# sin0235/FaceRecognition

Hardware: AMD Instinct MI355X
Metric: aligned faces/sec (embed+match) ArcFace@112 bs=256, 1/2/4/8 MI355X (higher is better)
Workload: dtype bf16; 1 GPU; iresnet100 bf16 embed bs=256/GPU + top-5 match vs 10000x512 f32 gallery (row-sharded over 1 GPU(s)); batch_per_gpu=256, global_batch=256, gallery_rows=10000, k=5, parallelism=dp1

## Files before the change

### facerecognition_amd/csrc/engine.cpp

```cpp
#include <algorithm>
#include <cmath>
#include <cstdio>
#include <cstdlib>
#include <cstring>
#include <memory>
#include <mutex>
#include <string>
#include <unordered_map>
#include <vector>

#include "engine_internal.h"

namespace fr {
static thread_local std::string g_err;
void set_error(const std::string& m) { g_err = m; }

static const std::vector<std::pair<std::string, std::string>>& ab_table() {
    static const std::vector<std::pair<std::string, std::string>> t = [] {
        std::vector<std::pair<std::string, std::string>> r;
        const char* e = getenv("FR_AB");
        const std::string v = e ? e : "";
        size_t p = 0;
        while (p < v.size()) {
            size_t q = v.find(',', p);
// ... 427 lines not shown
        h->stages.push_back(r);
    }
};

std::string L(int l, int i) { return "layer" + std::to_string(l) + "." + std::to_string(i); }

void build_iresnet100(Builder& b) {
    fr_handle* h = b.h;
    h->in_size = 112;
    const int in = b.tensor(112, 112, 8);
    h->ops.push_back(Op{OP_PRE, -1, 0, 0, in});
    int x = b.tensor(112, 112, 64, "prelu");
    b.stem = true;
    b.conv({"conv1"}, in, 0, 8, x, 0, 3, 3, 1, 1, 1, 1, 2);
    h->ops[h->ops.size() - 2].fuse_stem = true;
    const int planes[4] = {64, 128, 256, 512}, nblk[4] = {3, 13, 30, 3};
    int H = 112, C = 64;
    StageRec tail_rec;
    int tail_st_op = -1;
    for (int l = 0; l < 4; ++l) {
        const int P = planes[l], Ho = H / 2;
        int st_op = -1;
        StageRec rec;
        auto close_stage = [&](bool layer_end) {
            if (st_op >= 0 && !b.rc && layer_end && !rec.fp8 &&
                ((l == 2 && rec.parts == 1 && rec.C == 256) || (l == 1 && rec.parts == 2 && rec.C == 128 && rec.H == 28))) {
                rec.out = x;
                rec.nblk = (int)rec.t_tensors.size();
                tail_rec = rec;
                tail_st_op = st_op;
            } else if (st_op >= 0) {
                rec.out = x;
                rec.nblk = (int)rec.t_tensors.size();
                b.close_stage(st_op, rec);
            }
            st_op = -1;
        };
        for (int i = 0; i < nblk[l]; ++i) {
            const bool s14 = stage_supported(1, Ho, Ho, P);
            const int parts = split_stage_parts(Ho, Ho, P);
            const std::string pre = L(l + 1, i);
            const bool f8 = b.is_fp8(pre + ".conv1") && b.is_fp8(pre + ".conv2");
            const bool mixed = b.is_fp8(pre + ".conv1") != b.is_fp8(pre + ".conv2");
            const bool can = i >= 1 && P == C && !mixed && (f8 ? s14 : (s14 || parts > 0));
            if (st_op >= 0 && (!can || f8 != rec.fp8)) close_stage(false);
            if (can && st_op < 0) {
                st_op = b.open_stage();
                rec = StageRec{};
                rec.kind = STAGE_LDS;
                rec.in = x;
                rec.parts = s14 ? 1 : parts;
                rec.H = Ho;
                rec.C = P;
                rec.fp8 = f8;
            }
            const int Hin = i == 0 ? H : Ho, st = i == 0 ? 2 : 1;
            const bool fuse = i == 0 && b.fuse_ds(P, C, pre);
            const bool tr = i == 0 && fuse && !b.is_fp8(pre + ".conv1") && !b.is_fp8(pre + ".conv2") &&
                            trans_supported(1, H, H, C, P, P, 9 * C, 9 * P + C);
            const int tr_op = tr ? b.open_stage() : -1;
            const int hmid = b.tensor(Hin, Hin, P, pre + ".prelu");
            b.conv({pre + ".conv1"}, x, 0, C, hmid, 0, 3, 3, 1, 1, 1, 1, 2);
            if (tail_st_op >= 0 && !b.rc) {
                const int oi = (int)h->ops.size() - 1;
                const Op& op = h->ops[oi];
                const DevConvW& cw = h->convw[op.wi];
                static const bool no_tail = ab_int("no_stage_tail", 0) != 0;
                const int TC = tail_rec.C;
                if (!no_tail && h->dtype != FR_DTYPE_FP8 && !cw.w8 && op.act == 2 && cw.slope && cw.Cout == 2 * TC &&
                    cw.Npad >= 2 * TC && cw.Cin == TC && cw.Kh == 3 && cw.Kw == 3 && op.sh == 1 && op.sw == 1 && op.ph == 1 &&
                    op.pw == 1 && op.in == tail_rec.out && op.in_off == 0 && op.out_off == 0 && op.res < 0 && op.x2 < 0 &&
                    op.out2 < 0 && h->tensors[hmid].C == 2 * TC && !h->tensors[hmid].f16)
                    tail_rec.tail_op = oi;
                if (tail_rec.tail_op >= 0) tail_rec.conv_ops.push_back(oi);
                b.close_stage(tail_st_op, tail_rec);
                tail_st_op = -1;
            }
// ... 2 lines not shown
                res = b.tensor(Ho, Ho, P, pre + ".downsample");
                b.conv({pre + ".downsample"}, x, 0, C, res, 0, 1, 1, 2, 2, 0, 0, 0);
            }
            const int y = b.tensor(Ho, Ho, P, pre);
            if (fuse)
                b.conv_ds({pre + ".conv2"}, hmid, 0, P, y, 0, 3, 3, st, st, 1, 1, 0, -1, 0, -1, "", pre + ".downsample",
                          x, C, 2);
            else
                b.conv({pre + ".conv2"}, hmid, 0, P, y, 0, 3, 3, st, st, 1, 1, 0, res, 0);
            if (tr && !b.rc) {
                StageRec t;
                t.kind = STAGE_TRANS;
                t.in = x; t.out = y; t.nblk = 1; t.H = H; t.C = P;
                t.conv_ops = {(int)h->ops.size() - 2, (int)h->ops.size() - 1};
                t.t_tensors = {hmid};
                t.x_tensors = {y};
                b.close_stage(tr_op, t);
            }
            if (st_op >= 0 && !b.rc) {
                rec.conv_ops.push_back((int)h->ops.size() - 2);
                rec.conv_ops.push_back((int)h->ops.size() - 1);
                rec.t_tensors.push_back(hmid);
                rec.x_tensors.push_back(y);
            }
            x = y;
            C = P;
        }
        close_stage(true);
        H = Ho;
    }
    b.head(x);
}

int build_img_weights(fr_handle* h) {
    for (const auto& op : h->ops) {
        if (op.kind != OP_CONV || op.wi < 0) continue;
        DevConvW& cw = h->convw[op.wi];
        if ((cw.wimg || cw.wrows) && cw.wring) continue;
        ConvArgs a{};
        a.B = 1; a.Cin = op.cin; a.Kh = op.kh; a.Kw = op.kw; a.sh = op.sh; a.sw = op.sw; a.ph = op.ph; a.pw = op.pw;
        a.H = h->tensors[op.in].H; a.W = h->tensors[op.in].W; a.Cx = h->tensors[op.in].C; a.x_off = op.in_off;
        a.Ho = h->tensors[op.out].H; a.Wo = h->tensors[op.out].W; a.Cy = h->tensors[op.out].C; a.y_off = op.out_off;
        a.Cout = cw.Cout; a.Npad = cw.Npad; a.Kpad = cw.Kpad; a.bias9 = cw.bias9;
        a.y2 = op.out2 >= 0 ? (bf16_t*)1 : nullptr;
        if (op.res >= 0) { a.res = (const bf16_t*)1; a.Cres = h->tensors[op.res].C; a.res_off = op.res_off; }
        a.f16 = h->dtype == FR_DTYPE_F16;
// ... 334 lines not shown
        if ((rc = dev_alloc(&q, FR_SPLITK_TILES * sizeof(int)))) { free_acts(h); return rc; }
        h->act_allocs.push_back(q);
        FR_HIP_CHECK(hipMemset(q, 0, FR_SPLITK_TILES * sizeof(int)));
        h->splitk_cnt = (int*)q;
    }
    h->max_batch = maxB;
    if (std::any_of(h->need_amax.begin(), h->need_amax.end(), [](char c) { return c != 0; })) {
        void* q = nullptr;
        rc = dev_alloc(&q, h->tensors.size() * FR_AMAX_SLOTS * sizeof(float));
        if (rc) { free_acts(h); return rc; }
        h->act_allocs.push_back(q);
        h->amax = (float*)q;
    }
    if (h->proj_d) {
        void* q = nullptr;
        rc = dev_alloc(&q, (size_t)maxB * h->embed_dim * sizeof(float));
        if (rc) { free_acts(h); return rc; }
        h->act_allocs.push_back(q);
        h->emb_pre = (float*)q;
    }
    if (std::any_of(h->stages.begin(), h->stages.end(), [](const StageRec& r) { return r.parts > 1; })) {
        if (h->stages.size() > FR_MAX_SPLIT_STAGES) { set_error("reserve: too many stage ops"); return FR_ERR_ARG; }
        void* q = nullptr;
        rc = dev_alloc(&q, split_stage_xchg_elems(maxB) * sizeof(bf16_t));
        if (rc) { free_acts(h); return rc; }
        h->act_allocs.push_back(q);
        h->stage_xchg = (bf16_t*)q;
        rc = dev_alloc(&q, (size_t)maxB * 4 * FR_MAX_SPLIT_STAGES * sizeof(int));
        if (rc) { free_acts(h); return rc; }
        h->act_allocs.push_back(q);
        FR_HIP_CHECK(hipMemset(q, 0, (size_t)maxB * 4 * FR_MAX_SPLIT_STAGES * sizeof(int)));
        h->stage_flags = (int*)q;
    }
    return fill_stage_dbg(h);
}

bool img28_enabled() {
    static const bool on = [] { return !ab_int("no_img28", 0); }();
    return on;
}

bool rows_enabled() {
    static const bool on = [] { return !ab_int("no_rows", 0); }();
    return on;
}

bool img56_enabled() {
// ... 1172 lines not shown
        case FR_OPT_X3_MIN_ROWS:
            if (value < 1) { set_error("fr_set_option: FR_OPT_X3_MIN_ROWS must be >= 1"); return FR_ERR_ARG; }
            h->x3_min_rows = value;
            break;
        case FR_OPT_STAGE_SPIN_LIMIT: h->spin_limit = value; break;
        case FR_OPT_STAGE_VARIANT:
            if (value < 0 || value > 3) { set_error("fr_set_option: FR_OPT_STAGE_VARIANT is 0 .. 3"); return FR_ERR_ARG; }
            h->stage_variant = value;
            break;
        case FR_OPT_SPLITK_INLAUNCH: h->splitk_inlaunch = value != 0; break;
        case FR_OPT_BATCH_INVARIANT:
            if (value != 0 && h->dtype == FR_DTYPE_FP8) {
                set_error("fr_set_option: FR_OPT_BATCH_INVARIANT is not available on FR_DTYPE_FP8 handles (their e4m3 "
                          "convs scale activations by a per-batch amax)");
                return FR_ERR_ARG;
            }
            if ((value != 0) != h->invariant) {
                h->invariant = value != 0;
                h->tuned.clear();
                h->tuned_batches.clear();
            }
            break;
        case FR_OPT_FUSED_MASK:
            if (value < 0 || value > 127) { set_error("fr_set_option: FR_OPT_FUSED_MASK is 0 .. 127"); return FR_ERR_ARG; }
            h->fused_mask = value;
            break;
        default: set_error("fr_set_option: unknown option " + std::to_string(option)); return FR_ERR_ARG;
    }
    drop_graphs(h);
    return FR_OK;
}

int fr_get_option(const fr_handle* h, int option) {
    if (!h) return FR_ERR_ARG;
    switch (option) {
        case FR_OPT_STAGE: return h->stages.empty() ? 0 : h->stage_mode;
        case FR_OPT_STAGE_MIN_FILL: return h->stage_min_fill;
        case FR_OPT_KEEP_INTERMEDIATES: return h->keep_inter ? 1 : 0;
        case FR_OPT_MATCH_EXACT: return h->match_exact ? 1 : 0;
        case FR_OPT_X3_MIN_ROWS: return (int)h->x3_min_rows;
        case FR_OPT_STAGE_SPIN_LIMIT: return h->spin_limit;
        case FR_OPT_STAGE_VARIANT: return h->stage_variant;
        case FR_OPT_SPLITK_INLAUNCH: return h->splitk_inlaunch ? 1 : 0;
        case FR_OPT_BATCH_INVARIANT: return h->invariant ? 1 : 0;
        case FR_OPT_FUSED_MASK: return h->fused_mask;
        default: return FR_ERR_ARG;
    }
// ... 574 lines not shown
```

### facerecognition_amd/csrc/engine_internal.h

```cpp
#pragma once
#include <mutex>
#include <string>
#include <vector>

#include "../../include/frhip.h"
#include "kernels.h"

#pragma GCC visibility push(hidden)

namespace fr {

struct DevConvW {
    bf16_t* w = nullptr;
    float* bias = nullptr;
    float* slope = nullptr;
    float* aff_s = nullptr;
    float* aff_b = nullptr;
    float* bias9 = nullptr;
    bf16_t* wimg = nullptr;
    float* negf = nullptr;
    bf16_t* wrows = nullptr;
    float* ep = nullptr;
    bf16_t* wring = nullptr;
    uint8_t* w8 = nullptr;
// ... 16 lines not shown
    int in = -1, in_off = 0, cin = 0;
    int out = -1, out_off = 0;
    int res = -1, res_off = 0;
    int out2 = -1;
    int kh = 1, kw = 1, sh = 1, sw = 1, ph = 0, pw = 0;
    int act = 0;
    int wi = -1;
    int pk = 0, ps = 0, pp = 0;
    int stage = -1;
    int x2 = -1, x2_off = 0, st2 = 1;
    bool fuse_stem = false;
    int grp = -1;
};

enum StageKind {
    STAGE_LDS,
    STAGE_TRANS,
    STAGE_STEM160,
    STAGE_CHAIN35,
    STAGE_CHAIN17,
    STAGE_CHAIN_R50,
    STAGE_BNECK28,
    STAGE_STEM_R50,
    STAGE_NKINDS
};

struct StageRec {
    StageKind kind = STAGE_LDS;
    int in = -1, out = -1, nblk = 0;
    int parts = 1, H = 14, C = 256;
    std::vector<int> conv_ops;
    std::vector<int> t_tensors, x_tensors;
    bf16_t* w = nullptr;
    StageConv* table = nullptr;
    float* ep = nullptr;
    float* slope = nullptr;
    bf16_t** dbg = nullptr;
    bool fp8 = false;
    uint8_t* w8 = nullptr;
    float* wscale = nullptr;
    int tail_op = -1;
    bf16_t* tw1 = nullptr;
    bf16_t* tw2 = nullptr;
    float* tep1 = nullptr;
    float* tsl1 = nullptr;
    float* tb2 = nullptr;
// ... 68 lines not shown
    float* proj_b = nullptr;
    int proj_d = 0;
    float* emb_pre = nullptr;
    float* amax = nullptr;
    std::vector<char> need_amax;
    bf16_t* stage_xchg = nullptr;
    int* stage_flags = nullptr;
    int* stage_spin = nullptr;
    int* fail_host = nullptr;
    int* fail_dev = nullptr;
    int spin_limit = 0;
    int stage_variant = 0;
    bool no_split = false;
    int64_t stage_reruns = 0;
    hipEvent_t chk_ev = nullptr;
    hipEvent_t async_ev = nullptr;
    bool async_pending = false;
    bool split_registered = false;
    int stage_mode = 1;
    int stage_min_fill = 80;
    int n_cu = 256;
    bool keep_inter = false;
    bool invariant = false;
    int fused_mask = 127;
    const uint8_t* fwd_u8 = nullptr;
};

#pragma GCC visibility push(hidden)

namespace fr {

int dev_alloc(void** p, size_t bytes);

template <class T>
int upload(fr_handle* h, T** dst, const std::vector<T>& src) {
    void* p = nullptr;
    int rc = dev_alloc(&p, src.size() * sizeof(T));
    if (rc) return rc;
    h->weight_allocs.push_back(p);
    FR_HIP_CHECK(hipMemcpy(p, src.data(), src.size() * sizeof(T), hipMemcpyHostToDevice));
    *dst = (T*)p;
    return FR_OK;
}

int run_conv_op(fr_handle* h, const Op& op, int B, int f16, hipStream_t s);
int run_maxpool_op(fr_handle* h, const Op& op, int B, int f16, hipStream_t s);

// ... 62 lines not shown
```

### facerecognition_amd/csrc/kernels.h

```cpp
#pragma once
#include "common.h"

namespace fr {

enum { TILE_128x128 = 0, TILE_256x64 = 1, TILE_128x64 = 2, TILE_64x128 = 3,
       TILE_128x128_S3 = 4, TILE_256x128 = 5, TILE_128x256 = 6,
       TILE_128x64_S3 = 8, TILE_64x128_S3 = 9, NUM_TILE_IDS = 10,
       TILE_WRING = 13,
       TILE_DIRECT = 14,
       TILE_64x64_S3 = 17, TILE_64x64 = 18, TILE_32x64_S3 = 19 };

struct ConvArgs {
    const bf16_t* x; int B, H, W, Cx, x_off, Cin;
    const bf16_t* w; int Kh, Kw, sh, sw, ph, pw, K, Kpad;
    int Ho, Wo, M, Cout, Npad;
    const float* bias; const float* slope; int act;
    const float* bias9;
    const bf16_t* res; int Cres, res_off;
    bf16_t* y; int Cy, y_off;
    bf16_t* y2; int Cy2, y2_off; const float* aff_s; const float* aff_b;
    float* partial; int split_k;
    int f16;
    int tile;
    void* ev0;
// ... 69 lines not shown
    int* flags;
    int* spin_timeouts;
    int* fail_host;
    int spin_limit;
    int variant;
    int ntail;
    bf16_t* y2;
    int B, nblk, f16;
    void* ev0;
    void* ev1;
};
bool stage_supported(int B, int H, int W, int C);
size_t stage_weight_bytes(int nconv);
void stage_pack_weights(const bf16_t* rows, int Kpad, int C, bf16_t* out);
hipError_t launch_stage(const StageArgs& a, hipStream_t s);
size_t stage8_weight_bytes(int nconv);
void stage8_pack_weights(const uint8_t* rows, int Kpad8, uint8_t* out);
hipError_t launch_stage8(const StageArgs& a, hipStream_t s);
int split_stage_parts(int H, int W, int C);
size_t split_stage_weight_bytes(int C, int nconv);
void split_stage_pack_weights(const bf16_t* rows, int Kpad, int C, bf16_t* out);
size_t split_stage_xchg_elems(int B);
hipError_t launch_split_stage(const StageArgs& a, int H, int C, hipStream_t s);
struct TransArgs {
    const bf16_t* x;
    bf16_t* y;
    const bf16_t* w1;
    const bf16_t* w2;
    const float* ep1;
    const float* slope1;
    const float* b2;
    int B, f16;
    void* ev0;
    void* ev1;
};
bool trans_supported(int B, int H, int W, int Cin, int Cmid, int Cout, int K1, int K2);
size_t trans_packed_elems(int K);
hipError_t trans_pack_weights(const bf16_t* w, int Kpad, int K, bf16_t* out, hipStream_t s);
hipError_t launch_trans(const TransArgs& a, hipStream_t s);
struct Chain17Args {
    const bf16_t* x;
    bf16_t* y;
    const bf16_t* w;
    const float* bias;
    int B, nblk, f16;
    void* ev0;
// ... 130 lines not shown
```

### facerecognition_amd/csrc/stages.cpp

```cpp
#include <algorithm>
#include <cstdio>

#include "engine_internal.h"

namespace fr {

struct StageKindDesc {
    const char* name;
    int mask_bit;
    const char* ab_off[2];
    const char* ab_off_split;
    bool keeps_inter;
    bool no_amax;
    bool takes_u8;
    bool per_block;
    const char* cls;
    const char* label;
    const char* ksize;
    int pix, N, K;
    int K_ds;
};

static const StageKindDesc kinds[STAGE_NKINDS] = {
     {"stage", 1, {nullptr, nullptr}, "no_split_stage", true, false, false, false, nullptr, "stage", "3x3", 0, 0, 0, 0},
     {"transition", 1, {"no_trans", nullptr}, nullptr, false, true, false, false, "trans layer1.0", "trans", "3x3", 3136, 64, 2944, 0},
     {"stem160", 2, {"no_stem160", nullptr}, nullptr, false, false, true, false, "stem160", "stem160", "3x3", 1, 1, 185697536, 0},
     {"chain35", 4, {"no_chain", "no_chain35"}, nullptr, false, false, false, false, "chain block35", "chain", "3x3", 289, 256, 300, 0},
     {"chain", 8, {"no_chain", "no_chain17"}, nullptr, false, false, false, false, "chain block17", "chain", "1x1", 64, 896, 768, 0},
     {"chain_r50", 16, {"no_chain", "no_chain50"}, nullptr, false, false, false, false, "chain r50 layer3", "chain", "3x3", 49, 1024, 1088, 0},
     {"bneck28", 32, {"no_chain", "no_bneck28"}, nullptr, false, false, false, true, nullptr, "chain", "3x3", 784, 256, 272, 288},
     {"stem_r50", 64, {"no_chain", "no_stem_r50"}, nullptr, false, false, true, false, "stem r50", "chain", "7x7", 3136, 64, 392, 0},
};

struct StageWork {
    int pix, N, K, units;
};

static StageWork stage_work(const StageRec& r, int i) {
    const StageKindDesc& d = kinds[r.kind];
    StageWork w = {d.pix, d.N, d.K, r.nblk};
    if (!d.pix) w = {r.H * r.H, r.C, 9 * r.C, 2 * r.nblk};
    if (d.per_block && i >= 0) {
        w.units = 1;
        if (r.bn_ds && i == 0) w.K = d.K_ds;
    }
    return w;
}

static double stage_bytes(const fr_handle* h, const StageRec& r, const StageWork& w, int B, int i) {
    const double in_px = h->fwd_u8 ? 3.0 : 16.0;
    switch (r.kind) {
        case STAGE_TRANS: return 2.0 * B * (12544.0 + 3136.0) * 64 + 2.0 * 64 * (576 + 640);
        case STAGE_STEM160: return (double)B * (in_px * 160 * 160 + 2.0 * 38 * 38 * 80);
        case STAGE_STEM_R50: return (double)B * (112.0 * 112 * in_px + 28.0 * 28 * 64 * 2);
        case STAGE_BNECK28: return 2.0 * B * w.pix * ((r.bn_ds && i == 0 ? 64.0 : 256.0) + w.N) + 2.0 * w.N * w.K;
        default: return 2.0 * 2.0 * B * w.pix * w.N + (r.fp8 ? 1.0 : 2.0) * w.N * w.K * w.units;
    }
}

static const char* stage_class(const StageRec& r, int i) {
    switch (r.kind) {
        case STAGE_LDS: return r.fp8 ? "stage8 layer3" : r.H == 14 ? "stage layer3" : r.H == 28 ? "stage layer2" : "stage layer1";
        case STAGE_BNECK28: return r.bn_ds && i == 0 ? "bneck28 layer1.0" : "bneck28 layer1";
        default: return kinds[r.kind].cls;
// ... 83 lines not shown
        FR_HIP_CHECK(hipMemcpy(slope.data(), cw.slope, cw.Cout * sizeof(float), hipMemcpyDeviceToHost));
        for (int hf = 0; hf < 2; ++hf) {
            const int c = nconv + hf;
            if (r.parts > 1) split_stage_pack_weights(rows.data() + (size_t)hf * C * cw.Kpad, cw.Kpad, C, packed.data() + c * per);
            else stage_pack_weights(rows.data() + (size_t)hf * C * cw.Kpad, cw.Kpad, C, packed.data() + c * per);
            for (int k = 0; k < 9; ++k)
                std::copy(b9.begin() + (size_t)k * cw.Npad + hf * C, b9.begin() + (size_t)k * cw.Npad + hf * C + C,
                          ep.begin() + ((size_t)c * 9 + k) * C);
            std::copy(slope.begin() + hf * C, slope.begin() + hf * C + C, sl.begin() + (size_t)c * C);
        }
    }
    int rc = r.fp8 ? upload(h, &r.w8, packed8) : upload(h, &r.w, packed);
    if (rc) return rc;
    if (r.fp8 && (rc = upload(h, &r.wscale, wsc))) return rc;
    rc = upload(h, &r.table, tab);
    if (rc) return rc;
    if ((rc = upload(h, &r.ep, ep))) return rc;
    if ((rc = upload(h, &r.slope, sl))) return rc;
    void* d = nullptr;
    if ((rc = dev_alloc(&d, (size_t)nconv * sizeof(bf16_t*)))) return rc;
    h->weight_allocs.push_back(d);
    r.dbg = (bf16_t**)d;
    if (r.parts > 1 && !h->stage_spin) {
        if ((rc = dev_alloc(&d, sizeof(int)))) return rc;
        h->weight_allocs.push_back(d);
        h->stage_spin = (int*)d;
        FR_HIP_CHECK(hipMemset(h->stage_spin, 0, sizeof(int)));
    }
    return FR_OK;
}

int fill_stage_dbg(fr_handle* h) {
    for (auto& r : h->stages) {
        if (!kinds[r.kind].keeps_inter) continue;
        std::vector<bf16_t*> p(2 * r.nblk);
        for (int i = 0; i < r.nblk; ++i) {
            p[i] = h->tensors[r.x_tensors[i]].dev;
            p[r.nblk + i] = h->tensors[r.t_tensors[i]].dev;
        }
        FR_HIP_CHECK(hipMemcpy(r.dbg, p.data(), p.size() * sizeof(bf16_t*), hipMemcpyHostToDevice));
    }
    return FR_OK;
}

static int build_trans(fr_handle* h, StageRec& r) {
    const DevConvW& c1 = h->convw[h->ops[r.conv_ops[0]].wi];
// ... 176 lines not shown
        }
        bool shapes = cw[0]->Cout == 96 && cw[0]->K == 256 && cw[0]->Kh == 1 && cw[4]->Cout == 256 && cw[4]->K == 96 &&
                      cw[4]->Kh == 1 && op[4]->res >= 0 && op[4]->res_off == 0;
        for (int k = 1; k <= 3; ++k)
            shapes = shapes && cw[k]->Cout == 32 && cw[k]->K == 288 && cw[k]->Kh == 3 && cw[k]->Kw == 3 && op[k]->ph == 1 &&
                     op[k]->pw == 1 && op[k]->sh == 1 && op[k]->res < 0;
        if (!shapes) return bad_shapes("chain35 member convs do not have Block35's shapes");
        chain35_pack_block(m[0].rows.data(), cw[0]->Kpad, m[1].rows.data(), cw[1]->Kpad, m[2].rows.data(), cw[2]->Kpad,
                           m[3].rows.data(), cw[3]->Kpad, m[4].rows.data(), cw[4]->Kpad, blk, packed.data());
        chain35_pack_bias(m[0].bias.data(), m[1].bias.data(), m[2].bias.data(), m[3].bias.data(), m[4].bias.data(), blk,
                          bias.data());
    }
    return chain_upload(h, r, packed, bias);
}

int pack_stage(fr_handle* h, StageRec& r) {
    switch (r.kind) {
        case STAGE_LDS: return build_stage(h, r);
        case STAGE_TRANS: return build_trans(h, r);
        case STAGE_CHAIN35: return build_chain35(h, r);
        case STAGE_CHAIN17: return build_chain17(h, r);
        case STAGE_CHAIN_R50: return build_chain_r50(h, r);
        case STAGE_BNECK28: return build_bneck28(h, r);
        default: return FR_OK;
    }
}

int stage_choice(const fr_handle* h, int st, int B) {
    for (const auto& m : h->stage_meas)
        if (m.stage == st && m.B == B) return m.run;
    return -1;
}

static bool stage_runs(const fr_handle* h, int B, const StageRec& r, int st) {
    const StageKindDesc& d = kinds[r.kind];
    if (h->stage_mode == 0 || h->invariant) return false;
    if (!(h->fused_mask & d.mask_bit)) return false;
    if (h->keep_inter && !d.keeps_inter) return false;
    if (d.no_amax && h->amax && h->need_amax[r.out]) return false;
    if (!kind_enabled(r) || (r.parts > 1 && h->no_split)) return false;
    if (h->stage_mode == 1) {
        const int c = stage_choice(h, st, B);
        if (c >= 0) return c == 1;
    }
    const int cap = std::max(1, h->n_cu / r.parts);
    if (h->stage_mode == 2 || B <= cap) return true;
    const int64_t rounds = (B + cap - 1) / cap;
    return (int64_t)B * 100 >= (int64_t)h->stage_min_fill * rounds * cap;
}

std::vector<char> stage_plan(const fr_handle* h, int B) {
    std::vector<char> run(h->stages.size());
    for (size_t i = 0; i < h->stages.size(); ++i) run[i] = stage_runs(h, B, h->stages[i], (int)i);
    return run;
}

bool split_runs(const fr_handle* h, int B) {
    for (size_t i = 0; i < h->stages.size(); ++i)
        if (h->stages[i].parts > 1 && stage_runs(h, B, h->stages[i], (int)i)) return true;
    return false;
}

static hipError_t run_lds(fr_handle* h, const Op& op, const StageRec& r, int B, int f16, bool tail_in, hipStream_t s) {
    StageArgs a{};
    a.x = h->tensors[r.in].dev;
    a.y = h->tensors[r.out].dev;
    a.w = r.w;
    a.conv = r.table;
    a.ep = r.ep;
    a.slope = r.slope;
    if (h->keep_inter) { a.dbg_x = r.dbg; a.dbg_t = r.dbg + r.nblk; }
    a.B = B;
    a.nblk = r.nblk;
    a.f16 = f16;
    a.xchg = h->stage_xchg;
    a.flags = h->stage_flags + (size_t)h->max_batch * 4 * op.stage;
    a.spin_timeouts = h->stage_spin;
    a.fail_host = h->fail_dev;
    a.spin_limit = h->spin_limit;
    a.variant = h->stage_variant;
    if (tail_in) {
        a.ntail = 2;
        a.y2 = h->tensors[h->ops[r.tail_op].out].dev;
    }
    if (r.fp8) {
        a.w = (const bf16_t*)r.w8;
        a.wscale = r.wscale;
        return launch_stage8(a, s);
    }
    return r.parts > 1 ? launch_split_stage(a, r.H, r.C, s) : launch_stage(a, s);
}

static hipError_t run_trans(fr_handle* h, const StageRec& r, int B, int f16, hipStream_t s) {
    TransArgs t{};
    t.x = h->tensors[r.in].dev;
    t.y = h->tensors[r.out].dev;
    t.w1 = r.tw1; t.w2 = r.tw2; t.ep1 = r.tep1; t.slope1 = r.tsl1; t.b2 = r.tb2;
    t.B = B; t.f16 = f16;
    return launch_trans(t, s);
}

static hipError_t run_stem160(fr_handle* h, const StageRec& r, int B, int f16, hipStream_t s) {
    const DevConvW* cw[4];
    for (int k = 0, j = 0; k < 5; ++k)
        if (h->ops[r.conv_ops[k]].kind == OP_CONV) cw[j++] = &h->convw[h->ops[r.conv_ops[k]].wi];
    Stem160Args a{};
    a.x = h->tensors[r.in].dev;
    a.u8 = h->fwd_u8;
    a.y = h->tensors[r.out].dev;
    a.w1 = cw[0]->w; a.w2 = cw[1]->w; a.w3 = cw[2]->w; a.w4 = cw[3]->w;
    a.b1 = cw[0]->bias; a.b2 = cw[1]->bias; a.b3 = cw[2]->bias; a.b4 = cw[3]->bias;
    a.kp1 = cw[0]->Kpad; a.kp2 = cw[1]->Kpad; a.kp3 = cw[2]->Kpad; a.kp4 = cw[3]->Kpad;
// ... 35 lines not shown
    c.y = h->tensors[r.x_tensors[i]].dev;
    c.w = r.cw + (i ? bneck28_block_elems(r.bn_ds) + (size_t)(i - 1) * bneck28_block_elems(false) : 0);
    c.bias = r.cbias + 384 * i;
    return launch_bneck28(c, ds, s);
}

int run_stage(fr_handle* h, const Op& op, int B, int f16, const std::vector<char>& stage_run, hipStream_t s) {
    const StageRec& r = h->stages[op.stage];
    const int kf16 = f16 || h->tensors[r.in].f16;
    const bool tail_in = r.tail_op >= 0 && (r.parts > 1 || h->stage_variant != 1);
    const int nlaunch = kinds[r.kind].per_block ? r.nblk : 1;
    for (int i = 0; i < nlaunch; ++i) {
        const StageWork w = stage_work(r, i);
        ProfScope ps(h, s);
        ps.flops = 2.0 * B * w.pix * (double)w.N * w.K * w.units;
        ps.bytes = stage_bytes(h, r, w, B, i);
        if (tail_in) {
            ps.flops += 2.0 * B * w.pix * 2.0 * w.N * w.K;
            ps.bytes += 2.0 * B * w.pix * 2.0 * w.N + 2.0 * w.K * 2.0 * w.N;
        }
        ps.start(stage_class(r, i));
        hipError_t e = hipSuccess;
        switch (r.kind) {
            case STAGE_LDS: e = run_lds(h, op, r, B, kf16, tail_in, s); break;
            case STAGE_TRANS: e = run_trans(h, r, B, kf16, s); break;
            case STAGE_STEM160: e = run_stem160(h, r, B, kf16, s); break;
            case STAGE_CHAIN35: e = run_chain35(h, r, B, kf16, s); break;
            case STAGE_CHAIN17: e = launch_chain17(chain_args(h, r, B, kf16), s); break;
            case STAGE_CHAIN_R50: e = launch_chain_r50(chain_args(h, r, B, kf16), s); break;
            case STAGE_BNECK28: e = run_bneck28(h, r, B, kf16, i, s); break;
            case STAGE_STEM_R50: e = run_stem_r50(h, r, B, kf16, s); break;
            case STAGE_NKINDS: e = hipErrorInvalidValue; break;
        }
        FR_HIP_CHECK(e);
    }
    if (r.tail_op >= 0 && !tail_in) {
        const int rc = run_conv_op(h, h->ops[r.tail_op], B, f16, s);
        if (rc) return rc;
    }
    if (h->amax && h->need_amax[r.out] &&
        std::any_of(h->ops.begin(), h->ops.end(), [&](const Op& c) {
            return c.kind == OP_CONV && c.in == r.out && c.in_off == 0 && c.wi >= 0 && h->convw[c.wi].w8 &&
                   !op_skipped(c, stage_run);
        })) {
        const auto& t = h->tensors[r.out];
        ProfScope pa(h, s);
        pa.bytes = 2.0 * B * t.H * t.W * t.C;
// ... 63 lines not shown
```

Baseline: 51040 faces/s.

## Add fused pair7 stage kernel for layer4 512-channel 7x7 residual blocks

Adds a new persistent stage kind that fuses the last two layer4 residual blocks (four 3x3 512->512 convs at 7x7) into one kernel. Each workgroup handles two images and half the output channels, keeps the padded activation patch in LDS, and trades the other half's channels through a global exchange buffer guarded by spin flags. The kernel uses an MFMA weight ring, bank-conflict-checked pixel maps, and precomputed bias and PReLU tables. This is meant to cut per-conv launch cost and activation round-trips to global memory. In exchange it adds cross-workgroup spin synchronisation with a timeout path, and it becomes enabled by default through the fused mask change.

```diff
diff --git a/facerecognition_amd/csrc/conv_pair7.hip b/facerecognition_amd/csrc/conv_pair7.hip
--- /dev/null
+++ b/facerecognition_amd/csrc/conv_pair7.hip
@@ -0,0 +1,436 @@
+#include "kernels.h"
+
+#include <hip/hip_ext.h>
+
+#include <algorithm>
+#include <type_traits>
+
+namespace fr {
+namespace {
+
+constexpr int PW = 7;
+constexpr int PC = 512;
+constexpr int PH = 256;
+constexpr int PPIX = PW * PW;
+constexpr int NPX = 2 * PPIX;
+constexpr int PRS = 8;
+constexpr int PROWS = 17;
+constexpr int PPOS = PROWS * PRS;
+constexpr int PLANE_B = PPOS * 16;
+constexpr int NPL = PC / 8;
+constexpr int HPL = PH / 8;
+constexpr int LEAD_B = 256;
+constexpr int PATCH_B = NPL * PLANE_B;
+constexpr int TAIL_B = 256;
+constexpr int TROW = PH * 4 + 32;
+constexpr int TSL = 9 * TROW;
+constexpr int TS = TSL + PH * 4;
+constexpr int TAB = LEAD_B + PATCH_B + TAIL_B;
+constexpr int FAILED = TAB + 2 * TS;
+constexpr int PAIR7_LDS = FAILED + 16;
+constexpr int SLICE_B = 4 * PH * 16;
+constexpr int KSTEPS = (PC / 32) * 9;
+constexpr int NCONV = 4;
+constexpr int NW = 8;
+constexpr int FM = 7;
+constexpr int FN = 2;
+constexpr int NPW = 16 * FN;
+constexpr int RING = 6;
+constexpr int XHALF = HPL * NPX * 8;
+constexpr uint32_t OOB = 0x80000000u;
+constexpr int SPIN_LIMIT = 1 << 21;
+constexpr int SC1 = 16;
+constexpr int SPARE = 0xff;
+static_assert(PAIR7_LDS <= 163840, "LDS budget");
+static_assert(PLANE_B % 256 == 128, "plane stride = 8 bank slots mod 16");
+static_assert(18 % RING == 0 && KSTEPS % 18 == 0, "ring slot = K-step % RING is compile-time in the 18-step body");
+
+typedef __attribute__((address_space(3))) void lds_void;
+
+__device__ __forceinline__ int fresh_lane() {
+    int l;
+    asm volatile("v_mbcnt_lo_u32_b32 %0, -1, 0\n\tv_mbcnt_hi_u32_b32 %0, -1, %0" : "=v"(l));
+    return l;
+}
+__device__ __forceinline__ int opaque_tid() {
+    return (__builtin_amdgcn_readfirstlane(threadIdx.x) & ~63) + fresh_lane();
+}
+
+__host__ __device__ constexpr int prow(int i, int r) { return 1 + (PW + 1) * i + r; }
+__host__ __device__ constexpr int ppos(int i, int r, int c) { return prow(i, r) * PRS + c; }
+
+struct Map7 {
+    uint8_t pos[FM][16];
+    uint8_t cls[FM][16];
+    uint8_t pix[FM][16];
+};
+
+constexpr Map7 make_map7() {
+    Map7 m{};
+    for (int f = 0; f < FM; ++f)
+        for (int l = 0; l < 16; ++l) {
+            const int ra = 2 * f, rb = 2 * f + 1;
+            int row = 0, c = 0;
+            if (f == 3) {
+                row = (l >= 4 && l < 12) ? rb : ra;
+                c = l < 4 ? l : (l < 12 ? l - 4 : l - 8);
+            } else {
+                row = l < 8 ? ra : rb;
+                c = l < 4 ? 4 + l : (l < 8 ? l - 4 : (l < 12 ? l - 8 : l - 8));
+            }
+            const int i = row / PW, r = row % PW;
+            m.pos[f][l] = (uint8_t)ppos(i, r, c);
+            const bool real = c < PW;
+            m.cls[f][l] = (uint8_t)(real ? 3 * (r == 0 ? 0 : (r == PW - 1 ? 2 : 1)) + (c == 0 ? 0 : (c == PW - 1 ? 2 : 1)) : SPARE);
+            m.pix[f][l] = (uint8_t)(real ? i * PPIX + r * PW + c : SPARE);
+        }
+    return m;
+}
+__constant__ Map7 kMap7 = make_map7();
+
+constexpr bool map7_ok() {
+    constexpr Map7 m = make_map7();
+    const int X[8] = {0, 1, 2, 3, 12, 13, 14, 15}, Y[8] = {4, 5, 6, 7, 8, 9, 10, 11};
+    for (int f = 0; f < FM; ++f)
+        for (int swap = 0; swap < 2; ++swap) {
+            bool seen[16] = {};
+            for (int k = 0; k < 8; ++k) {
+                const int a = (swap ? Y : X)[k], b = (swap ? X : Y)[k];
+                const int sa = m.pos[f][a] % 16, sb = (PPOS + m.pos[f][b]) % 16;
+                if (seen[sa]) return false;
+                seen[sa] = true;
+                if (seen[sb]) return false;
+                seen[sb] = true;
+            }
+        }
+    int owned[NPX] = {};
+    for (int f = 0; f < FM; ++f)
+        for (int l = 0; l < 16; ++l) {
+            const int q = m.pos[f][l];
+            if (q - PRS - 1 < -1 || q + PRS + 1 > PPOS) return false;
+            if (m.pix[f][l] == SPARE) {
+                if (q % PRS != PW) return false;
+                continue;
+            }
+            const int i = m.pix[f][l] / PPIX, r = m.pix[f][l] % PPIX / PW, c = m.pix[f][l] % PW;
+            if (q != ppos(i, r, c)) return false;
+            ++owned[m.pix[f][l]];
+        }
+    for (int k = 0; k < NPX; ++k)
+        if (owned[k] != 1) return false;
+    return true;
+}
+static_assert(map7_ok(), "pair stage map: bank conflict, tap out of the plane or pixel not owned exactly once");
+
+__host__ __device__ constexpr int step_cg(int s, int half) { return (s / 9 + (PC / 64) * half) % (PC / 32); }
+__host__ __device__ constexpr int step_tap(int s) { return s % 9; }
+constexpr int OWN_STEPS = KSTEPS / 2;
+constexpr bool steps_ok(int half) {
+    int seen[9][PC / 32] = {};
+    for (int s = 0; s < KSTEPS; ++s) {
+        ++seen[step_tap(s)][step_cg(s, half)];
+        if ((s < OWN_STEPS) != (step_cg(s, half) / (PC / 64) == half)) return false;
+    }
+    for (int t = 0; t < 9; ++t)
+        for (int g = 0; g < PC / 32; ++g)
+            if (seen[t][g] != 1) return false;
+    return true;
+}
+static_assert(steps_ok(0) && steps_ok(1), "pair stage K-step order");
+
+template <bool F16>
+__global__ __launch_bounds__(64 * NW, 1) void pair7_kernel(StageArgs p) {
+    typedef Num<F16> T;
+    typedef typename T::frag frag;
+    extern __shared__ __attribute__((aligned(16))) char smem[];
+    const int lane = threadIdx.x & 63;
+    const int wave = __builtin_amdgcn_readfirstlane(threadIdx.x >> 6);
+    const int blk = blockIdx.x;
+    const int q = blk / 16 * 8 + (blk & 7), half = (blk >> 3) & 1;
+    if (2 * q >= p.B) return;
+    const int nimg = min(2, p.B - 2 * q);
+    char* const patch = smem + LEAD_B;
+    constexpr int total = NCONV * KSTEPS;
+
+    const __amdgpu_buffer_rsrc_t wr = __builtin_amdgcn_make_buffer_rsrc(
+        (void*)(p.w + (size_t)half * total * (SLICE_B / 2)), 0, (uint32_t)total * SLICE_B, 0x00020000);
+
+    {
+        const __amdgpu_buffer_rsrc_t xr = __builtin_amdgcn_make_buffer_rsrc(
+            (void*)(p.x + (size_t)2 * q * PPIX * PC), 0, (uint32_t)(nimg * PPIX * PC * 2), 0x00020000);
+        for (int u = 0; u < PATCH_B / 1024 / NW; ++u) {
+            const int piece = wave + NW * u, s = piece * 64 + lane;
+            const int plane = s / PPOS, pos = s - plane * PPOS, R = pos / PRS, c = pos % PRS;
+            const int i = R > PW + 1, r = R - prow(i, 0);
+            const uint32_t src = c < PW && (unsigned)r < (unsigned)PW ? (uint32_t)((((i * PPIX + r * PW + c) * PC) + plane * 8) * 2) : OOB;
+            __builtin_amdgcn_raw_ptr_buffer_load_lds(xr, (lds_void*)(patch + piece * 1024), 16, src, 0, 0, 0);
+        }
+        static_assert(PATCH_B % (1024 * NW) == 0, "patch pieces per wave");
+        if (threadIdx.x < (LEAD_B + TAIL_B) / 16)
+            *(uint4*)(threadIdx.x < LEAD_B / 16 ? smem + threadIdx.x * 16 : patch + PATCH_B + (threadIdx.x - LEAD_B / 16) * 16) =
+                make_uint4(0, 0, 0, 0);
+        if (threadIdx.x == 0) *(int*)(smem + FAILED) = 0;
+    }
+    int aoff[FM];
+#pragma unroll
+    for (int j = 0; j < FM; ++j) aoff[j] = (lane >> 4) * PLANE_B + kMap7.pos[j][lane & 15] * 16;
+    const uint32_t wvo = (uint32_t)((lane >> 4) * (PH * 16) + (wave * NPW + (lane & 15)) * 16);
+
+    f32x4_t acc[FN][FM];
+    frag pA[FM];
+    const int cg_own = (PC / 64) * half;
+    auto pread = [&](frag (&pf)[FM], int cg, int tap) {
+        const char* pa = patch + ((cg + cg_own) & (PC / 32 - 1)) * 4 * PLANE_B + ((tap / 3 - 1) * PRS + tap % 3 - 1) * 16;
+#pragma unroll
+        for (int j = 0; j < FM; ++j) pf[j] = *(const frag*)(pa + aoff[j]);
+    };
+    frag wq[RING][FN];
+    auto wload = [&](frag (&w)[FN], int g) {
+#pragma unroll
+        for (int i = 0; i < FN; ++i)
+            w[i] = __builtin_bit_cast(frag, __builtin_amdgcn_raw_buffer_load_b128(wr, wvo + i * 256, (uint32_t)g * SLICE_B, 0));
+    };
+    auto kstep1 = [&](int g, int r, frag (&pf)[FM], int cg_n, int tap_n) {
+        asm volatile("" ::: "memory");
+        __builtin_amdgcn_sched_barrier(0);
+        wload(wq[(r + RING - 1) % RING], g + RING - 1 < total ? g + RING - 1 : total - 1);
+        const char* pa = patch + ((cg_n + cg_own) & (PC / 32 - 1)) * 4 * PLANE_B + ((tap_n / 3 - 1) * PRS + tap_n % 3 - 1) * 16;
+#pragma unroll
+        for (int j = 0; j < FM; ++j) {
+#pragma unroll
+            for (int i = 0; i < FN; ++i) acc[i][j] = T::mfma(wq[r][i], pf[j], acc[i][j]);
+            pf[j] = *(const frag*)(pa + aoff[j]);
+        }
+        __builtin_amdgcn_sched_group_barrier(0x020, FN, 0);
+#pragma unroll
+        for (int s = 0; s < FM; ++s) {
+            __builtin_amdgcn_sched_group_barrier(0x008, FN, 0);
+            __builtin_amdgcn_sched_group_barrier(0x100, 1, 0);
+        }
+    };
+
+    const __amdgpu_buffer_rsrc_t epr = __builtin_amdgcn_make_buffer_rsrc(
+        (void*)(p.ep + (size_t)half * NCONV * 9 * PH), 0, (uint32_t)(NCONV * 9 * PH * 4), 0x00020000);
+    const __amdgpu_buffer_rsrc_t slr = __builtin_amdgcn_make_buffer_rsrc(
+        (void*)(p.slope + (size_t)half * NCONV * PH), 0, (uint32_t)(NCONV * PH * 4), 0x00020000);
+    auto issue_tab = [&](int cv, int cv_slope, int slot) {
+        char* dst = smem + TAB + slot * TS;
+        const int ln = fresh_lane();
+#pragma unroll
+        for (int u = 0; u < 2; ++u) {
+            const int piece = wave + NW * u;
+            if (piece < 9)
+                __builtin_amdgcn_raw_ptr_buffer_load_lds(epr, (lds_void*)(dst + piece * TROW), 16,
+                                                         (uint32_t)(piece * 1024 + ln * 16), (uint32_t)(cv * 9 * PH * 4), 0, 0);
+        }
+        if (cv_slope >= 0 && wave == NW - 1)
+            __builtin_amdgcn_raw_ptr_buffer_load_lds(slr, (lds_void*)(dst + TSL), 16, (uint32_t)(ln * 16),
+                                                     (uint32_t)(cv_slope * PH * 4), 0, 0);
+    };
+    auto tab_row = [&](int j) {
+        const int pos = (aoff[j] >> 4) % PPOS, R = pos >> 3, c = pos & 7, r = R > PW + 1 ? R - prow(1, 0) : R - prow(0, 0);
+        return (3 * (r == 0 ? 0 : (r == PW - 1 ? 2 : 1)) + (c == 0 ? 0 : (c == PW - 1 ? 2 : 1))) * TROW;
+    };
+    auto seed_bias = [&](int slot) {
+        const int ln = fresh_lane();
+        const char* t = smem + TAB + slot * TS + (wave * NPW + 4 * (ln >> 4)) * 4;
+#pragma unroll
+        for (int j = 0; j < FM; ++j) {
+            const int tr = tab_row(j);
+#pragma unroll
+            for (int i = 0; i < FN; ++i) {
+                const float4 bb = *(const float4*)(t + tr + 64 * i);
+                acc[i][j] = (f32x4_t){bb.x, bb.y, bb.z, bb.w};
+            }
+        }
+    };
+
+    const int spin_limit = p.spin_limit > 0 ? p.spin_limit : (p.spin_limit == 0 ? SPIN_LIMIT : 0);
+    int* const my_flag = p.flags + 2 * q + half;
+    const int* const nf = p.flags + 2 * q + (1 - half);
+    const int f0 = __hip_atomic_load(my_flag, __ATOMIC_RELAXED, __HIP_MEMORY_SCOPE_AGENT);
+    const __amdgpu_buffer_rsrc_t xr_x = __builtin_amdgcn_make_buffer_rsrc(
+        (void*)(p.xchg + (size_t)q * 4 * XHALF), 0, (uint32_t)(4 * XHALF * 2), 0x00020000);
+    auto publish = [&](int cv) __attribute__((always_inline)) {
+        const int par = cv & 1;
+        for (int c = opaque_tid(); c < HPL * NPX; c += 64 * NW) {
+            const int pl = c / NPX, px = c - pl * NPX, i = px / PPIX, r = (px - i * PPIX) / PW, col = px % PW;
+            const uint4 v = *(const uint4*)(patch + (half * HPL + pl) * PLANE_B + ppos(i, r, col) * 16);
+            typedef unsigned u32x4 __attribute__((ext_vector_type(4)));
+            __builtin_amdgcn_raw_buffer_store_b128((u32x4){v.x, v.y, v.z, v.w}, xr_x,
+                                                   (uint32_t)(((half * 2 + par) * XHALF + c * 8) * 2), 0, SC1);
+        }
+        asm volatile("s_waitcnt vmcnt(0)\n\ts_barrier" ::: "memory");
+        if (threadIdx.x == 0)
+            __hip_atomic_store(my_flag, (int)((unsigned)f0 + (unsigned)(cv + 1)), __ATOMIC_RELAXED, __HIP_MEMORY_SCOPE_AGENT);
+    };
+    auto import_issue = [&](int cv) __attribute__((always_inline)) {
+        const int par = cv & 1;
+        if (wave == 0 && lane == 0) {
+            int it = 0;
+            while (p.spin_limit < 0 ||
+                   (int)((unsigned)__hip_atomic_load(nf, __ATOMIC_RELAXED, __HIP_MEMORY_SCOPE_AGENT) - (unsigned)f0) < cv + 1) {
+                if (it++ >= spin_limit) {
+                    __hip_atomic_fetch_add(p.spin_timeouts, 1, __ATOMIC_RELAXED, __HIP_MEMORY_SCOPE_AGENT);
+                    *(volatile int*)p.fail_host = 1;
+                    *(volatile int*)(smem + FAILED) = 1;
+                    asm volatile("s_waitcnt vmcnt(0) lgkmcnt(0)" ::: "memory");
+                    break;
+                }
+                __builtin_amdgcn_s_sleep(1);
+            }
+        }
+        asm volatile("s_barrier" ::: "memory");
+        const int ln = fresh_lane();
+#pragma unroll
+        for (int u = 0; u < 2 * HPL / NW; ++u) {
+            const int idx = wave + NW * u, pl = idx >> 1, seg = idx & 1;
+            const int pos = PRS + seg * 64 + ln, R = pos / PRS, c = pos % PRS;
+            const int i = R > PW + 1, r = R - prow(i, 0);
+            const uint32_t off = c < PW && (unsigned)r < (unsigned)PW
+                                     ? (uint32_t)(((((1 - half) * 2 + par) * XHALF) + (pl * NPX + i * PPIX + r * PW + c) * 8) * 2)
+                                     : OOB;
+            char* dst = patch + ((1 - half) * HPL + pl) * PLANE_B + (PRS + seg * 64) * 16;
+            if (pos < (PROWS - 1) * PRS)
+                __builtin_amdgcn_raw_ptr_buffer_load_lds(xr_x, (lds_void*)dst, 16, off, 0, 0, SC1);
+        }
+    };
+    int pending = -1;
+
+    issue_tab(0, -1, 0);
+    asm volatile("s_waitcnt vmcnt(0)" ::: "memory");
+    __syncthreads();
+#pragma unroll
+    for (int s = 0; s < RING - 1; ++s) wload(wq[s], s);
+
+    constexpr int IMPORT_CG = 2, LAND_CG = 6;
+    static_assert(LAND_CG * 9 + 18 <= OWN_STEPS && IMPORT_CG < LAND_CG, "the import lands under own-half K-steps");
+    auto kloop = [&](int cv) __attribute__((always_inline)) {
+        pread(pA, 0, 0);
+        const int g0 = cv * KSTEPS;
+#pragma unroll 1
+        for (int cg = 0; cg < PC / 32; cg += 2) {
+            if (pending >= 0 && cg == IMPORT_CG) import_issue(pending);
+            if (pending >= 0 && cg == LAND_CG) {
+                asm volatile("s_waitcnt vmcnt(0)\n\ts_barrier" ::: "memory");
+                pending = -1;
+            }
+#pragma unroll
+            for (int t = 0; t < 18; ++t) {
+                const int cgn = cg + (t + 1) / 9, tapn = (t + 1) % 9;
+                kstep1(g0 + cg * 9 + t, t % RING, pA, cgn, tapn);
+            }
+        }
+    };
+    auto copy_out = [&](bf16_t* yo, uint32_t nan_or) __attribute__((always_inline)) {
+        constexpr int NIT = (NPX + 15) / 16 * 16 * HPL;
+        for (int c = opaque_tid(); c < NIT; c += 64 * NW) {
+            const int rr = c >> 6, px = (rr / (HPL / 4)) * 16 + (c & 15), pl = (rr % (HPL / 4)) * 4 + ((c >> 4) & 3);
+            const int i = px / PPIX;
+            if (px >= NPX || i >= nimg) continue;
+            const int pix = px - i * PPIX;
+            uint4 v = *(const uint4*)(patch + (half * HPL + pl) * PLANE_B + ppos(i, pix / PW, pix % PW) * 16);
+            v.x |= nan_or; v.y |= nan_or; v.z |= nan_or; v.w |= nan_or;
+            *(uint4*)(yo + ((size_t)(2 * q + i) * PPIX + pix) * PC + (half * HPL + pl) * 8) = v;
+        }
+    };
+    auto run_conv = [&](int cv, auto second_tag) __attribute__((always_inline)) {
+        constexpr bool second = decltype(second_tag)::value;
+        if (!second) {
+            seed_bias(0);
+            if (cv + 1 < NCONV) issue_tab(cv + 1, cv, 1);
+        } else if (cv + 1 < NCONV) {
+            issue_tab(cv + 1, -1, 0);
+        }
+        kloop(cv);
+        asm volatile("s_waitcnt lgkmcnt(0)\n\ts_barrier" ::: "memory");
+        {
+            const int ln = fresh_lane();
+            const int g = ln >> 4;
+            const char* t2 = smem + TAB + TS;
+            const int cb = (half * HPL + NPW / 8 * wave + (g >> 1) - g) * PLANE_B + (g & 1) * 8;
+#pragma unroll
+            for (int j = 0; j < FM; ++j) {
+                char* const sj = patch + aoff[j] + cb;
+                const int tr = second ? 0 : tab_row(j);
+                const bool real = ((aoff[j] >> 4) & 7) != PW;
+#pragma unroll
+                for (int i = 0; i < FN; ++i) {
+                    const int n = wave * NPW + 16 * i + 4 * g;
+                    char* const slot = sj + 2 * i * PLANE_B;
+                    float v[4] = {acc[i][j][0], acc[i][j][1], acc[i][j][2], acc[i][j][3]};
+                    if (!second) {
+                        const float4 sl = *(const float4*)(t2 + TSL + n * 4);
+                        v[0] = fmaf(sl.x - 1.f, min0_raw(v[0]), v[0]);
+                        v[1] = fmaf(sl.y - 1.f, min0_raw(v[1]), v[1]);
+                        v[2] = fmaf(sl.z - 1.f, min0_raw(v[2]), v[2]);
+                        v[3] = fmaf(sl.w - 1.f, min0_raw(v[3]), v[3]);
+                    }
+                    float o8[8] = {v[0], v[1], v[2], v[3], 0, 0, 0, 0};
+                    const uint4 pk = T::pack8(o8);
+                    if (!second) {
+                        const uint2 xin = *(const uint2*)slot;
+                        float f[8];
+                        T::unpack8(make_uint4(xin.x, xin.y, 0, 0), f);
+                        const float4 bb = *(const float4*)(t2 + tr + n * 4);
+                        acc[i][j] = (f32x4_t){f[0] + bb.x, f[1] + bb.y, f[2] + bb.z, f[3] + bb.w};
+                    }
+                    if (real) *(uint2*)slot = make_uint2(pk.x, pk.y);
+                }
+            }
+        }
+        asm volatile("s_waitcnt lgkmcnt(0)\n\ts_barrier" ::: "memory");
+        bf16_t* dbg = nullptr;
+        if (p.dbg_x) dbg = second ? p.dbg_x[cv >> 1] : p.dbg_t[cv >> 1];
+        const bool last = cv == NCONV - 1;
+        if (last) {
+            const uint32_t nan_or = *(const volatile int*)(smem + FAILED) ? 0x7FC07FC0u : 0u;
+            copy_out(p.y, nan_or);
+            if (dbg && dbg != p.y) copy_out(dbg, 0u);
+        } else {
+            if (dbg) copy_out(dbg, 0u);
+            publish(cv);
+            pending = cv;
+        }
+    };
+#pragma unroll 1
+    for (int blkc = 0; blkc < NCONV / 2; ++blkc) {
+        run_conv(2 * blkc, std::false_type{});
+        run_conv(2 * blkc + 1, std::true_type{});
+    }
+    asm volatile("s_waitcnt vmcnt(0)" ::: "memory");
+}
+
+}
+
+bool pair7_supported(int H, int W, int C) { return H == PW && W == PW && C == PC; }
+
+size_t pair7_weight_elems() { return (size_t)2 * NCONV * KSTEPS * (SLICE_B / 2); }
+
+size_t pair7_xchg_elems(int B) { return (size_t)((B + 1) / 2) * 4 * XHALF; }
+
+void pair7_pack_weights(const bf16_t* rows, int Kpad, int conv, int half, bf16_t* out) {
+    bf16_t* o = out + ((size_t)half * NCONV + conv) * KSTEPS * (SLICE_B / 2);
+    for (int s = 0; s < KSTEPS; ++s) {
+        const int cg = step_cg(s, half), tap = step_tap(s);
+        bf16_t* d = o + (size_t)s * (SLICE_B / 2);
+        for (int g = 0; g < 4; ++g)
+            for (int n = 0; n < PH; ++n)
+                for (int e = 0; e < 8; ++e)
+                    d[(g * PH + n) * 8 + e] = rows[(size_t)(half * PH + n) * Kpad + tap * PC + cg * 32 + g * 8 + e];
+    }
+}
+
+hipError_t launch_pair7(const StageArgs& a, hipStream_t s) {
+    if (a.B <= 0 || a.nblk != 2 || !a.xchg || !a.flags || !a.spin_timeouts || !a.fail_host) return hipErrorInvalidValue;
+    auto k = a.f16 ? pair7_kernel<true> : pair7_kernel<false>;
+    if (hipError_t e = lds_opt_in((const void*)k, PAIR7_LDS); e != hipSuccess) return e;
+    const dim3 grid(((a.B + 1) / 2 + 7) / 8 * 16);
+    if (a.ev0)
+        hipExtLaunchKernelGGL(k, grid, dim3(64 * NW), PAIR7_LDS, s, (hipEvent_t)a.ev0, (hipEvent_t)a.ev1, 0, a);
+    else
+        hipLaunchKernelGGL(k, grid, dim3(64 * NW), PAIR7_LDS, s, a);
+    return hipGetLastError();
+}
+
+}
diff --git a/facerecognition_amd/csrc/engine.cpp b/facerecognition_amd/csrc/engine.cpp
--- a/facerecognition_amd/csrc/engine.cpp
+++ b/facerecognition_amd/csrc/engine.cpp
@@ -473,6 +473,9 @@
         const int P = planes[l], Ho = H / 2;
         int st_op = -1;
         StageRec rec;
+        int pair_op = -1;
+        bool pair_fits = true;
+        StageRec pair_rec;
         auto close_stage = [&](bool layer_end) {
             if (st_op >= 0 && !b.rc && layer_end && !rec.fp8 &&
                 ((l == 2 && rec.parts == 1 && rec.C == 256) || (l == 1 && rec.parts == 2 && rec.C == 128 && rec.H == 28))) {
@@ -504,6 +507,15 @@
                 rec.H = Ho;
                 rec.C = P;
                 rec.fp8 = f8;
+            }
+            if (l == 3 && i == 1 && nblk[l] == 3 && h->dtype != FR_DTYPE_FP8 && pair7_supported(Ho, Ho, P) && !b.rc) {
+                pair_op = b.open_stage();
+                pair_rec = StageRec{};
+                pair_rec.kind = STAGE_PAIR7;
+                pair_rec.in = x;
+                pair_rec.parts = 2;
+                pair_rec.H = Ho;
+                pair_rec.C = P;
             }
             const int Hin = i == 0 ? H : Ho, st = i == 0 ? 2 : 1;
             const bool fuse = i == 0 && b.fuse_ds(P, C, pre);
@@ -552,6 +564,28 @@
                 rec.conv_ops.push_back((int)h->ops.size() - 1);
                 rec.t_tensors.push_back(hmid);
                 rec.x_tensors.push_back(y);
+            }
+            if (pair_op >= 0 && !b.rc) {
+                for (int k = 2; k >= 1; --k) {
+                    const int oi = (int)h->ops.size() - k;
+                    const Op& op = h->ops[oi];
+                    const DevConvW& cw = h->convw[op.kind == OP_CONV && op.wi >= 0 ? op.wi : 0];
+                    pair_fits = pair_fits && op.kind == OP_CONV && op.wi >= 0 && !cw.w8 && cw.Cout == P && cw.Cin == P && cw.Npad >= P &&
+                                cw.Kh == 3 && cw.Kw == 3 && op.sh == 1 && op.sw == 1 && op.ph == 1 && op.pw == 1 &&
+                                op.in_off == 0 && op.out_off == 0 && op.x2 < 0 && op.out2 < 0 &&
+                                (k == 2 ? op.act == 2 && cw.slope && op.res < 0 && op.in == x
+                                        : op.act == 0 && op.res == x && op.res_off == 0 && op.in == hmid) &&
+                                !h->tensors[op.in].f16 && !h->tensors[op.out].f16;
+                    pair_rec.conv_ops.push_back(oi);
+                }
+                pair_rec.t_tensors.push_back(hmid);
+                pair_rec.x_tensors.push_back(y);
+                if (i == nblk[l] - 1) {
+                    pair_rec.out = y;
+                    pair_rec.nblk = (int)pair_rec.t_tensors.size();
+                    b.close_stage(pair_op, pair_rec, pair_fits && P == 512 && pair_rec.nblk == 2);
+                    pair_op = -1;
+                }
             }
             x = y;
             C = P;
@@ -932,7 +966,7 @@
     if (std::any_of(h->stages.begin(), h->stages.end(), [](const StageRec& r) { return r.parts > 1; })) {
         if (h->stages.size() > FR_MAX_SPLIT_STAGES) { set_error("reserve: too many stage ops"); return FR_ERR_ARG; }
         void* q = nullptr;
-        rc = dev_alloc(&q, split_stage_xchg_elems(maxB) * sizeof(bf16_t));
+        rc = dev_alloc(&q, std::max(split_stage_xchg_elems(maxB), pair7_xchg_elems(maxB)) * sizeof(bf16_t));
         if (rc) { free_acts(h); return rc; }
         h->act_allocs.push_back(q);
         h->stage_xchg = (bf16_t*)q;
@@ -2151,7 +2185,7 @@
             }
             break;
         case FR_OPT_FUSED_MASK:
-            if (value < 0 || value > 127) { set_error("fr_set_option: FR_OPT_FUSED_MASK is 0 .. 127"); return FR_ERR_ARG; }
+            if (value < 0 || value > 255) { set_error("fr_set_option: FR_OPT_FUSED_MASK is 0 .. 255"); return FR_ERR_ARG; }
             h->fused_mask = value;
             break;
         default: set_error("fr_set_option: unknown option " + std::to_string(option)); return FR_ERR_ARG;
diff --git a/facerecognition_amd/csrc/engine_internal.h b/facerecognition_amd/csrc/engine_internal.h
--- a/facerecognition_amd/csrc/engine_internal.h
+++ b/facerecognition_amd/csrc/engine_internal.h
@@ -62,6 +62,7 @@
     STAGE_CHAIN_R50,
     STAGE_BNECK28,
     STAGE_STEM_R50,
+    STAGE_PAIR7,
     STAGE_NKINDS
 };
 
@@ -176,7 +177,7 @@
     int n_cu = 256;
     bool keep_inter = false;
     bool invariant = false;
-    int fused_mask = 127;
+    int fused_mask = 255;
     const uint8_t* fwd_u8 = nullptr;
 };
 
diff --git a/facerecognition_amd/csrc/kernels.h b/facerecognition_amd/csrc/kernels.h
--- a/facerecognition_amd/csrc/kernels.h
+++ b/facerecognition_amd/csrc/kernels.h
@@ -115,6 +115,11 @@
 void split_stage_pack_weights(const bf16_t* rows, int Kpad, int C, bf16_t* out);
 size_t split_stage_xchg_elems(int B);
 hipError_t launch_split_stage(const StageArgs& a, int H, int C, hipStream_t s);
+bool pair7_supported(int H, int W, int C);
+size_t pair7_weight_elems();
+size_t pair7_xchg_elems(int B);
+void pair7_pack_weights(const bf16_t* rows, int Kpad, int conv, int half, bf16_t* out);
+hipError_t launch_pair7(const StageArgs& a, hipStream_t s);
 struct TransArgs {
     const bf16_t* x;
     bf16_t* y;
diff --git a/facerecognition_amd/csrc/stages.cpp b/facerecognition_amd/csrc/stages.cpp
--- a/facerecognition_amd/csrc/stages.cpp
+++ b/facerecognition_amd/csrc/stages.cpp
@@ -30,6 +30,7 @@
      {"chain_r50", 16, {"no_chain", "no_chain50"}, nullptr, false, false, false, false, "chain r50 layer3", "chain", "3x3", 49, 1024, 1088, 0},
      {"bneck28", 32, {"no_chain", "no_bneck28"}, nullptr, false, false, false, true, nullptr, "chain", "3x3", 784, 256, 272, 288},
      {"stem_r50", 64, {"no_chain", "no_stem_r50"}, nullptr, false, false, true, false, "stem r50", "chain", "7x7", 3136, 64, 392, 0},
+     {"pair7", 128, {"no_pair7", nullptr}, nullptr, true, true, false, false, "pair layer4", "pair", "3x3", 49, 512, 4608, 0},
 };
 
 struct StageWork {
@@ -40,6 +41,7 @@
     const StageKindDesc& d = kinds[r.kind];
     StageWork w = {d.pix, d.N, d.K, r.nblk};
     if (!d.pix) w = {r.H * r.H, r.C, 9 * r.C, 2 * r.nblk};
+    if (r.kind == STAGE_PAIR7) w.units = 2 * r.nblk;
     if (d.per_block && i >= 0) {
         w.units = 1;
         if (r.bn_ds && i == 0) w.K = d.K_ds;
@@ -169,6 +171,56 @@
     h->weight_allocs.push_back(d);
     r.dbg = (bf16_t**)d;
     if (r.parts > 1 && !h->stage_spin) {
+        if ((rc = dev_alloc(&d, sizeof(int)))) return rc;
+        h->weight_allocs.push_back(d);
+        h->stage_spin = (int*)d;
+        FR_HIP_CHECK(hipMemset(h->stage_spin, 0, sizeof(int)));
+    }
+    return FR_OK;
+}
+
+static int bad_shapes(const char* what);
+
+static int build_pair7(fr_handle* h, StageRec& r) {
+    constexpr int nconv = 4, C = 512, HC = 256;
+    if (r.nblk != 2 || (int)r.conv_ops.size() != nconv || r.parts != 2) return bad_shapes("pair7 member count");
+    std::vector<bf16_t> packed(pair7_weight_elems());
+    std::vector<float> ep((size_t)2 * nconv * 9 * HC, 0.f), sl((size_t)2 * nconv * HC, 0.f);
+    for (int c = 0; c < nconv; ++c) {
+        const Op& op = h->ops[r.conv_ops[c]];
+        const DevConvW& cw = h->convw[op.wi];
+        if (cw.w8 || cw.Cout != C || cw.Npad < C || cw.Kh != 3 || cw.Kw != 3 || cw.Cin != C || cw.Kpad < 9 * C)
+            return bad_shapes("pair7 member conv is not a bf16 / f16 3x3 512->512");
+        if ((c % 2 == 0 && (op.act != 2 || !cw.slope)) || (c % 2 == 1 && (op.act != 0 || op.res < 0)))
+            return bad_shapes("pair7 member conv has an unexpected activation / residual");
+        std::vector<bf16_t> rows((size_t)cw.Npad * cw.Kpad);
+        FR_HIP_CHECK(hipMemcpy(rows.data(), cw.w, rows.size() * sizeof(bf16_t), hipMemcpyDeviceToHost));
+        std::vector<float> b9((size_t)9 * C, 0.f), slope(C, 1.f);
+        if (cw.bias9) {
+            for (int k = 0; k < 9; ++k)
+                FR_HIP_CHECK(hipMemcpy(b9.data() + (size_t)k * C, cw.bias9 + (size_t)k * cw.Npad, C * sizeof(float), hipMemcpyDeviceToHost));
+        } else if (cw.bias) {
+            FR_HIP_CHECK(hipMemcpy(b9.data(), cw.bias, C * sizeof(float), hipMemcpyDeviceToHost));
+            for (int k = 1; k < 9; ++k) std::copy(b9.begin(), b9.begin() + C, b9.begin() + (size_t)k * C);
+        }
+        if (op.act == 2) FR_HIP_CHECK(hipMemcpy(slope.data(), cw.slope, C * sizeof(float), hipMemcpyDeviceToHost));
+        for (int hf = 0; hf < 2; ++hf) {
+            pair7_pack_weights(rows.data(), cw.Kpad, c, hf, packed.data());
+            for (int k = 0; k < 9; ++k)
+                std::copy(b9.begin() + (size_t)k * C + hf * HC, b9.begin() + (size_t)k * C + hf * HC + HC,
+                          ep.begin() + (((size_t)hf * nconv + c) * 9 + k) * HC);
+            std::copy(slope.begin() + hf * HC, slope.begin() + hf * HC + HC, sl.begin() + ((size_t)hf * nconv + c) * HC);
+        }
+    }
+    int rc = upload(h, &r.w, packed);
+    if (rc) return rc;
+    if ((rc = upload(h, &r.ep, ep))) return rc;
+    if ((rc = upload(h, &r.slope, sl))) return rc;
+    void* d = nullptr;
+    if ((rc = dev_alloc(&d, (size_t)nconv * sizeof(bf16_t*)))) return rc;
+    h->weight_allocs.push_back(d);
+    r.dbg = (bf16_t**)d;
+    if (!h->stage_spin) {
         if ((rc = dev_alloc(&d, sizeof(int)))) return rc;
         h->weight_allocs.push_back(d);
         h->stage_spin = (int*)d;
@@ -391,6 +443,7 @@
         case STAGE_CHAIN17: return build_chain17(h, r);
         case STAGE_CHAIN_R50: return build_chain_r50(h, r);
         case STAGE_BNECK28: return build_bneck28(h, r);
+        case STAGE_PAIR7: return build_pair7(h, r);
         default: return FR_OK;
     }
 }
@@ -412,7 +465,7 @@
         const int c = stage_choice(h, st, B);
         if (c >= 0) return c == 1;
     }
-    const int cap = std::max(1, h->n_cu / r.parts);
+    const int cap = std::max(1, r.kind == STAGE_PAIR7 ? h->n_cu : h->n_cu / r.parts);
     if (h->stage_mode == 2 || B <= cap) return true;
     const int64_t rounds = (B + cap - 1) / cap;
     return (int64_t)B * 100 >= (int64_t)h->stage_min_fill * rounds * cap;
@@ -457,6 +510,7 @@
         a.wscale = r.wscale;
         return launch_stage8(a, s);
     }
+    if (r.kind == STAGE_PAIR7) return launch_pair7(a, s);
     return r.parts > 1 ? launch_split_stage(a, r.H, r.C, s) : launch_stage(a, s);
 }
 
@@ -538,7 +592,8 @@
         ps.start(stage_class(r, i));
         hipError_t e = hipSuccess;
         switch (r.kind) {
-            case STAGE_LDS: e = run_lds(h, op, r, B, kf16, tail_in, s); break;
+            case STAGE_LDS:
+            case STAGE_PAIR7: e = run_lds(h, op, r, B, kf16, tail_in, s); break;
             case STAGE_TRANS: e = run_trans(h, r, B, kf16, s); break;
             case STAGE_STEM160: e = run_stem160(h, r, B, kf16, s); break;
             case STAGE_CHAIN35: e = run_chain35(h, r, B, kf16, s); break;
```

Result: no change. 51110 faces/s, median of 2 (+0.1%).
